# komxun/gym-pybullet-drones-routing

Hardware: AMD Instinct MI355X
Metric: env-steps/sec (drone·dt) at 4096 envs, 1/2/4/8 GPU; state L2 vs PyBullet (higher is better)
Workload: dtype f64; 1 GPU; 4096 HoverAviary envs per GPU (cf2x, Physics.DYN, ActionType.RPM, 240/30 Hz = 8 substeps/step, U[-1,1] actions, SB3 auto-reset); n_envs_per_gpu=4096, global_envs=4096, drones_per_env=1, parallelism=env-sharded x1 (no collective in the step loop)

## Files before the change

### gym_pybullet_drones_routing_amd/csrc/gpd_step_seq.h

```cpp
#pragma once
#include "gpd_step_duo.h"

namespace gpd {


__host__ __device__ inline int seq_rows(int nsub) { return (5 * nsub + 3) | 1; }
__host__ __device__ inline int seq_hand_off_at(int tile_bytes) { return (tile_bytes + 15) & ~15; }
inline size_t seq_lds_bytes(int tile_bytes, int nsub, int tpb, size_t real_bytes) {
  return (size_t)seq_hand_off_at(tile_bytes) + (size_t)2 * 2 * seq_rows(nsub) * tpb * real_bytes;
}

template <typename R, int ACT>
__global__ __launch_bounds__(4 * kWave) void step_seq_kernel(R* __restrict__ state_p, const float* __restrict__ actions_p,
                                                             int2* __restrict__ ctr_p, const Consts<R>* __restrict__ cp,
                                                             long long npad_p, int n_p, int tpb_p, SimView<R> v,
                                                             StepIO<R> io, int n_slots, int slot0, int n_steps,
                                                             int hand_off_at) {
  static_assert(!act_is_pid(ACT), "the fused sequence kernel serves the RPM action types");
  v.state = state_p; v.ctr = ctr_p; v.npad = npad_p; v.N = n_p; v.tpb = tpb_p;
  constexpr int A = act_width(ACT);
  extern __shared__ float4 tile4[];
  float* tilef = reinterpret_cast<float*>(tile4);
  __shared__ unsigned long long sdone[2];
  __shared__ unsigned long long sreset[2];
  __shared__ int shead[kWave];
  const Consts<R>& c = *cp;
  const int tid = threadIdx.x & (kWave - 1);
  const int wave = __builtin_amdgcn_readfirstlane(threadIdx.x) / kWave;
  const long long n0 = (long long)blockIdx.x * v.tpb;
  const long long n = n0 + tid;
  const int nact = (int)((v.N - n0) < v.tpb ? (v.N - n0) : v.tpb);
  const bool active = tid < nact;
  const long long nn = active ? n : n0;
  const long long slot_stride = (long long)v.N * A;
  int slot = slot0;
  auto next_slot = [&]() { slot = slot + 1 == n_slots ? 0 : slot + 1; };
  float nxt[A];
  R* const hbuf = reinterpret_cast<R*>(reinterpret_cast<char*>(tile4) + hand_off_at);
  const int rows = seq_rows(c.nsub);
  const int cstride = v.tpb * rows;
  const int pstride = 2 * cstride;
  const bool own = tid < v.tpb;
  const int lrow = (own ? tid : 0) * rows;

  if (wave == 2) {
    const int L = v.ring_len;
    {
      const float* rb = v.ring + ridx(nn, 0, L, A);
      for (int s = 0; s < L; ++s) {
        const float* src = rb + (long long)s * (64 * A);
        if (A == 4) __builtin_amdgcn_global_load_lds((gbl_void_ptr)src, (lds_void_ptr)(tile4 + s * kPad), 16, 0, 0);
        else __builtin_amdgcn_global_load_lds((gbl_void_ptr)src, (lds_void_ptr)(tilef + s * kPad), 4, 0, 0);
      }
    }
    int hd = v.ctr[nn].y;
    action_load<A>(actions_p + slot * slot_stride, nn, nxt);
    asm volatile("s_waitcnt vmcnt(0)" ::: "memory");
    shead[tid] = hd;
    wave_lds_sync();
    constexpr int U = 4;
    constexpr int EB = A == 4 ? 16 : 4;
    const int total = nact * L;
    const int NC = A == 4 ? 3 + L : v.W;
    const int c0 = A == 4 ? 3 : 12;
    const float rL = 1.0f / (float)L;
    const bool fits = total <= U * kWave;
    const bool wt_rows = (v.wt & 1) != 0;
    const int span = L * kPad;
    float* const dst0 = uniform_ptr(io.obs + n0 * v.W);
    const int nrec = __builtin_amdgcn_readfirstlane(nact * v.W * 4);
    const __amdgpu_buffer_rsrc_t rsrc = __builtin_amdgcn_make_buffer_rsrc(dst0, 0, nrec, 0x00020000);
    int off[U], row[U], idx[U];
#pragma unroll
    for (int u = 0; u < U; ++u) {
      const int g = tid + u * kWave;
      const bool ok = g < total;
      const int gg = ok ? g : total - 1;
      const int i = (int)(((float)gg + 0.5f) * rL), k = gg - i * L;
      int s = shead[i] + 1 + k;
      s -= s >= L ? L : 0;
      s -= s >= L ? L : 0;
      row[u] = i;
      off[u] = ok ? (i * NC + c0 + k) * EB : nrec;
      idx[u] = s * kPad + i;
    }
    int tmod = 0;
    asm volatile("s_barrier" ::: "memory");
    for (int t = 0; t < n_steps; ++t) {
      float a[A];
#pragma unroll
      for (int j = 0; j < A; ++j) a[j] = nxt[j];
      next_slot();
      if (t + 1 < n_steps) action_load<A>(actions_p + slot * slot_stride, nn, nxt);
      if (A == 4) tile4[hd * kPad + tid] = make_float4(a[0], a[1], a[2], a[3]);
      else tilef[hd * kPad + tid] = a[0];
      if (active) ring_append<A>(v.ring, n, hd, L, a);
      wave_lds_sync();
      float4 v4[U];
      float v1[U];
      if (fits) {
#pragma unroll
        for (int u = 0; u < U; ++u) {
          if (A == 4) v4[u] = tile4[idx[u]];
          else v1[u] = tilef[idx[u]];
        }
#pragma unroll
        for (int u = 0; u < U; ++u) {
          if (wt_rows) {
            if (A == 4) store_wt(rsrc, off[u], v4[u]);
            else store_wt(rsrc, off[u], v1[u]);
          } else {
            if (A == 4) __builtin_amdgcn_raw_buffer_store_b128(__builtin_bit_cast(gpd_v4i, v4[u]), rsrc, off[u], 0, 0);
            else __builtin_amdgcn_raw_buffer_store_b32(__builtin_bit_cast(unsigned, v1[u]), rsrc, off[u], 0, 0);
          }
        }
      }
      for (int g = fits ? total : tid; g < total; g += kWave) {
        const int i = (int)(((float)g + 0.5f) * rL), k = g - i * L;
        int s = shead[i] + tmod + 1 + k;
        s -= s >= L ? L : 0;
        s -= s >= L ? L : 0;
        const int o = (i * NC + c0 + k) * EB;
        if (A == 4) {
          const float4 p = tile4[s * kPad + i];
          if (wt_rows) store_wt(rsrc, o, p);
          else __builtin_amdgcn_raw_buffer_store_b128(__builtin_bit_cast(gpd_v4i, p), rsrc, o, 0, 0);
        } else {
          const float p = tilef[s * kPad + i];
          if (wt_rows) store_wt(rsrc, o, p);
          else __builtin_amdgcn_raw_buffer_store_b32(__builtin_bit_cast(unsigned, p), rsrc, o, 0, 0);
        }
      }
      lds_barrier();
      const unsigned long long dr = sdone[t & 1];
      if (dr) {
        float* const tdst = io.terminal_obs + n0 * v.W;
        if (fits) {
#pragma unroll
          for (int u = 0; u < U; ++u) {
            if (tid + u * kWave < total && ((dr >> row[u]) & 1ull)) {
              char* const tp = reinterpret_cast<char*>(tdst) + off[u];
              if (A == 4) *reinterpret_cast<float4*>(tp) = v4[u];
              else *reinterpret_cast<float*>(tp) = v1[u];
            }
          }
        }
        for (int g = fits ? total : tid; g < total; g += kWave) {
          const int i = (int)(((float)g + 0.5f) * rL), k = g - i * L;
          if ((dr >> i) & 1ull) {
            int s = shead[i] + tmod + 1 + k;
            s -= s >= L ? L : 0;
            s -= s >= L ? L : 0;
            const int e = i * NC + c0 + k;
            if (A == 4) reinterpret_cast<float4*>(tdst)[e] = tile4[s * kPad + i];
            else tdst[e] = tilef[s * kPad + i];
          }
        }
      }
      hd = hd + 1 == L ? 0 : hd + 1;
      tmod = tmod + 1 == L ? 0 : tmod + 1;
#pragma unroll
      for (int u = 0; u < U; ++u) {
        idx[u] += kPad;
        idx[u] -= idx[u] >= span ? span : 0;
      }
    }
    return;
  }

  const R* st = v.state + tidx(nn, 0, kStateComps);

  if (wave != 0) {
    const bool from_zero = wave == 3;
    R* const hw = hbuf + (from_zero ? cstride : 0) + lrow;
    if (from_zero) next_slot();
    if (!from_zero || n_steps > 1) action_load<A>(actions_p + slot * slot_stride, nn, nxt);
    R wx = R(0), wy = R(0), wz = R(0);
    if (!from_zero) { wx = st[10 * 64]; wy = st[11 * 64]; wz = st[12 * 64]; }
    DynK<R> dk = dyn_consts(c);
    const int nsub = dk.nsub;
    asm volatile("" : "+v"(wx), "+v"(wy), "+v"(wz));
    auto chain = [&](int u, R* out) {
      float a[A];
#pragma unroll
      for (int j = 0; j < A; ++j) a[j] = nxt[j];
      next_slot();
      if (u + 1 < n_steps) action_load<A>(actions_p + slot * slot_stride, nn, nxt);
      R rpm[4], W[4];
#pragma unroll
      for (int k = 0; k < 4; ++k) rpm[k] = (R)action_to_rpm(dk.hover_f32, a[A == 4 ? k : 0]);
      rpm_wrench<R, 0>(rpm, dk, c, W);
      rate_recur(wx, wy, wz, W, dk);
      for (int k = 0; k < nsub - 1; ++k) {
        R h[5], n2;
        const R cx = wx, cy = wy, cz = wz;
        const bool big = rate_weights(cx, cy, cz, dk, h, n2);
        rate_weights_big(big, n2, dk, h);
        if (own) {
#pragma unroll
          for (int j = 0; j < 5; ++j) out[5 * k + j] = h[j];
        }
        rate_recur(wx, wy, wz, W, dk);
      }
      {
        R h[5], n2;
        const bool big = rate_weights(wx, wy, wz, dk, h, n2);
        rate_weights_big(big, n2, dk, h);
        if (own) {
          R* const o = out + 5 * (nsub - 1);
#pragma unroll
          for (int j = 0; j < 5; ++j) o[j] = h[j];
          o[5] = wx; o[6] = wy; o[7] = wz;
        }
      }
    };
    for (int t = -1; t < n_steps; ++t) {
      if (t + 1 < n_steps && (t >= 0 || !from_zero)) {
        if (from_zero) {
          wx = wy = wz = R(0);
          asm volatile("" : "+v"(wx), "+v"(wy), "+v"(wz));
        } else if (t > 0) {
          if ((sreset[(t - 1) & 1] >> tid) & 1ull) {
            const R* e = hbuf + (t & 1) * pstride + cstride + lrow + 5 * nsub;
            wx = e[0]; wy = e[1]; wz = e[2];
          }
        }
        chain(t + 1, hw + ((t + 1) & 1) * pstride);
      }
      lds_barrier();
    }
    return;
  }

  action_load<A>(actions_p + slot * slot_stride, nn, nxt);
  Drone<R> s;
  R last[4];
  load_drone(v, nn, s, last, false);
  const int2 cv = v.ctr[nn];
  int sc = cv.x;
  int head = cv.y;
  DynK<R> dk = dyn_consts(c, v.task, io.trunc);
  const TailK<R> tk = tail_consts(c, v.bound_xy);
  const int nsub = dk.nsub;
  gpd_global R* st_out = (gpd_global R*)(v.state + tidx(nn, 0, kStateComps));
  int st_off = (int)(tidx(nn, 0, kStateComps) * sizeof(R));
  gpd_global float* rew_out = (gpd_global float*)(io.reward + nn);
  gpd_global uint8_t* term_out = (gpd_global uint8_t*)(io.term + nn);
  gpd_global uint8_t* trunc_out = (gpd_global uint8_t*)(io.trunc + nn);
  gpd_global gpd_v2i* ctr_out = (gpd_global gpd_v2i*)(v.ctr + nn);
  asm volatile("" : "+v"(st_out), "+v"(st_off), "+v"(rew_out), "+v"(term_out), "+v"(trunc_out), "+v"(ctr_out));
  asm volatile("" : "+v"(s.px), "+v"(s.py), "+v"(s.pz), "+v"(s.qx), "+v"(s.qy), "+v"(s.qz), "+v"(s.qw), "+v"(s.vx),
               "+v"(s.vy), "+v"(s.vz), "+v"(sc), "+v"(head));
  const R wnone[3] = {R(0), R(0), R(0)};
  auto hand_off = [&](const R* hp, int k, R h[5]) {
#pragma unroll
    for (int j = 0; j < 5; ++j) h[j] = hp[5 * k + j];
  };
  bool was_reset = false;
  lds_barrier();
  for (int t = 0; t < n_steps; ++t) {
    float a[A];
#pragma unroll
    for (int j = 0; j < A; ++j) a[j] = nxt[j];
    next_slot();
    if (t + 1 < n_steps) action_load<A>(actions_p + slot * slot_stride, nn, nxt);
    R fz;
    {
      R rpm[4], W[4];
#pragma unroll
      for (int k = 0; k < 4; ++k) rpm[k] = (R)action_to_rpm(dk.hover_f32, a[A == 4 ? k : 0]);
      rpm_wrench<R, 0>(rpm, dk, c, W);
      fz = W[0];
#pragma unroll
      for (int k = 0; k < 4; ++k) last[k] = rpm[k];
    }
    const R* const hp = hbuf + (t & 1) * pstride + (was_reset ? cstride : 0) + lrow;
    R h[5];
    hand_off(hp, 0, h);
    if (nsub > 1) {
      R hn[5];
      hand_off(hp, 1, hn);
      pose_half<R, false, true>(s, fz, h, wnone, dk);
      for (int k = 1; k < nsub - 1; ++k) {
#pragma unroll
        for (int j = 0; j < 5; ++j) h[j] = hn[j];
        hand_off(hp, k + 1, hn);
        pose_half<R, false, false>(s, fz, h, wnone, dk);
      }
#pragma unroll
      for (int j = 0; j < 5; ++j) h[j] = hn[j];
    }
    {
      const R* const e = hp + 5 * nsub;
      s.wx = e[0]; s.wy = e[1]; s.wz = e[2];
      const R w[3] = {s.wx, s.wy, s.wz};
      if (nsub > 1) pose_half<R, true, false, true>(s, fz, h, w, dk);
      else pose_half<R, true, true>(s, fz, h, w, dk);
    }
    R qn[4], Rm[9];
    if constexpr (sizeof(R) == 8) readback_fused_rare(s.qx, s.qy, s.qz, s.qw, qn, Rm);
    else readback_fused(s.qx, s.qy, s.qz, s.qw, qn, Rm);
    AttitudeArgs<R> att = attitude_args(qn);
    bool tilted, up_unused;
    attitude_decide<R, true, false>(s.qx, s.qy, s.qz, s.qw, att, tilted, up_unused);
    float roll, pitch, yaw;
    obs_euler_f32(qn, att, roll, pitch, yaw);
    float reward = -1.0f;
    bool term = false, trunc = false;
    if (v.task != TASK_NONE) {
      const R tx = tk.tg[0] - s.px, ty = tk.tg[1] - s.py, tz = tk.tg[2] - s.pz;
      const R d2 = hover_d2(tx, ty, tz);
      R r = R(2) - d2 * d2;
      r = r > R(0) ? r : R(0);
      const bool oob = g_abs(s.px) > tk.bound_xy || g_abs(s.py) > tk.bound_xy || s.pz > R(2) || tilted;
      reward = (float)r;
      term = d2 < R(0.99e-8);
      const bool band = !(d2 < R(0.99e-8)) && !(d2 > R(1.01e-8));
      if (GPD_RARE(__ballot(band) != 0ull)) term = g_sqrt(d2) < R(1e-4);
      trunc = oob || sc >= v.trunc_sc;
    }
    const bool done = term || trunc;
    const bool do_reset = done && v.autoreset;
    float row12[12] = {(float)s.px, (float)s.py, (float)s.pz, roll, pitch, yaw,
                       (float)s.vx, (float)s.vy, (float)s.vz, (float)s.ax, (float)s.ay, (float)s.az};
    if (do_reset) {
      if (active && io.terminal_obs != nullptr) row12_store<A>(io.terminal_obs + n * v.W, row12);
      reset_to_template(tk.ini, s, last, row12);
    }
    const unsigned long long done_rows = __ballot(do_reset && active && io.terminal_obs != nullptr);
    const unsigned long long reset_rows = __ballot(do_reset);
    if (active) {
      if (A == 4) {
        const float4 r0 = make_float4(row12[0], row12[1], row12[2], row12[3]);
        const float4 r1 = make_float4(row12[4], row12[5], row12[6], row12[7]);
        const float4 r2 = make_float4(row12[8], row12[9], row12[10], row12[11]);
        if (v.wt & 1) {
          const __amdgpu_buffer_rsrc_t r =
              __builtin_amdgcn_make_buffer_rsrc(io.obs + n0 * v.W, 0, nact * v.W * 4, 0x00020000);
          const int o = tid * v.W * 4;
          store_wt(r, o, r0); store_wt(r, o + 16, r1); store_wt(r, o + 32, r2);
        } else {
          float4* o4 = reinterpret_cast<float4*>(io.obs + n * v.W);
          o4[0] = r0; o4[1] = r1; o4[2] = r2;
        }
      } else {
        float* orow = io.obs + n * v.W;
#pragma unroll
        for (int k = 0; k < 12; ++k) orow[k] = row12[k];
      }
    }
    if (tid == 0) { sdone[t & 1] = done_rows; sreset[t & 1] = reset_rows; }
    was_reset = do_reset;
    lds_barrier();
    if (active) {
      *rew_out = reward;
      *term_out = (uint8_t)(term ? 1 : 0);
      *trunc_out = (uint8_t)(trunc ? 1 : 0);
    }
    sc = do_reset ? 0 : sc + nsub;
    head = head + 1 == v.ring_len ? 0 : head + 1;
  }
  if (!active) return;
  store_drone_step_at<R, kAuxWt>(v, st_out, st_off, s, last);
  mark_last_in_ring_single(v, n);
  *ctr_out = gpd_v2i{sc, head};
}

}
```

Baseline: 15.01 billion drone*dt/s.

## Offload obs/reward/flag writes to ring wave and reuse precomputed thrust

The pose wave no longer computes Euler angles, builds the observation row, or writes reward/term/trunc. It stages raw state, attitude args and reward in a new double-buffered LDS row buffer, and the ring wave (wave 2) converts and stores them. The thrust fz is now written into the hand-off rows by the rate waves instead of being recomputed from actions in the critical pose wave, and the final rpm is recomputed only once after the loop. This shortens the serial pose-wave chain at the cost of more LDS, another cross-wave dependency and f64-only specialisation.

```diff
diff --git a/gym_pybullet_drones_routing_amd/csrc/gpd_step_seq.h b/gym_pybullet_drones_routing_amd/csrc/gpd_step_seq.h
--- a/gym_pybullet_drones_routing_amd/csrc/gpd_step_seq.h
+++ b/gym_pybullet_drones_routing_amd/csrc/gpd_step_seq.h
@@ -4,10 +4,52 @@
 namespace gpd {
 
 
-__host__ __device__ inline int seq_rows(int nsub) { return (5 * nsub + 3) | 1; }
+__host__ __device__ inline int seq_rows(int nsub) { return (5 * nsub + 4) | 1; }
+constexpr int kSeqRowVals = 18;
 __host__ __device__ inline int seq_hand_off_at(int tile_bytes) { return (tile_bytes + 15) & ~15; }
+__host__ __device__ inline int seq_row_buf_at(int nsub, int tpb) { return 2 * 2 * seq_rows(nsub) * tpb; }
 inline size_t seq_lds_bytes(int tile_bytes, int nsub, int tpb, size_t real_bytes) {
-  return (size_t)seq_hand_off_at(tile_bytes) + (size_t)2 * 2 * seq_rows(nsub) * tpb * real_bytes;
+  return (size_t)seq_hand_off_at(tile_bytes) +
+         ((size_t)seq_row_buf_at(nsub, tpb) + (size_t)2 * kSeqRowVals * tpb) * real_bytes;
+}
+
+__device__ __forceinline__ double seq_rate_n2(double wx, double wy, double wz) {
+#pragma clang fp contract(off)
+  return __builtin_fma(wz, wz, __builtin_fma(wy, wy, wx * wx));
+}
+__device__ __forceinline__ void seq_yaw_args(const double q[4], double& yn, double& yd) {
+#pragma clang fp contract(off)
+  const double x = q[0], y = q[1], z = q[2], w = q[3];
+  yn = 2.0 * __builtin_fma(x, y, w * z);
+  yd = ((w * w + x * x) - y * y) - z * z;
+}
+template <typename R>
+__device__ __forceinline__ bool seq_rate_weights(R wx, R wy, R wz, const DynK<R>& k, R h[5], R& n2) {
+  n2 = seq_rate_n2(wx, wy, wz);
+  const bool rot = n2 > R(1e-16);
+  const R t2 = n2 * k.hdt2;
+  R co, sc;
+  cos_sinc(t2, co, sc);
+  h[0] = co; h[1] = k.hdt * sc;
+  h[2] = rot ? wx : R(0); h[3] = rot ? wy : R(0); h[4] = rot ? wz : R(0);
+  return t2 >= R(0.25);
+}
+
+template <typename R>
+__device__ __forceinline__ void seq_obs_euler_f32(R sarg, R a, R b, R yn, R yd, R x, R y, float& roll, float& pitch,
+                                                  float& yaw) {
+  const bool gimbal = sarg <= R(-0.99999) || sarg >= R(0.99999);
+  const R sa = sarg < R(-1) ? R(-1) : (sarg > R(1) ? R(1) : sarg);
+  pitch = asinf((float)sa);
+  roll = atan2f((float)a, (float)b);
+  yaw = atan2f((float)yn, (float)yd);
+  if (GPD_RARE(__ballot(gimbal) != 0ull)) {
+    if (sarg <= R(-0.99999)) {
+      pitch = -1.57079632679489661923f; roll = 0.0f; yaw = (float)(R(2) * g_atan2(x, -y));
+    } else if (sarg >= R(0.99999)) {
+      pitch = 1.57079632679489661923f; roll = 0.0f; yaw = (float)(R(2) * g_atan2(-x, y));
+    }
+  }
 }
 
 template <typename R, int ACT>
@@ -17,12 +59,15 @@
                                                              StepIO<R> io, int n_slots, int slot0, int n_steps,
                                                              int hand_off_at) {
   static_assert(!act_is_pid(ACT), "the fused sequence kernel serves the RPM action types");
+  static_assert(sizeof(R) == 8, "the fused sequence kernel is built for f64 sims only (gpd.hip, step_seq_fn)");
   v.state = state_p; v.ctr = ctr_p; v.npad = npad_p; v.N = n_p; v.tpb = tpb_p;
   constexpr int A = act_width(ACT);
   extern __shared__ float4 tile4[];
   float* tilef = reinterpret_cast<float*>(tile4);
   __shared__ unsigned long long sdone[2];
   __shared__ unsigned long long sreset[2];
+  __shared__ unsigned long long sterm[2];
+  __shared__ unsigned long long strunc[2];
   __shared__ int shead[kWave];
   const Consts<R>& c = *cp;
   const int tid = threadIdx.x & (kWave - 1);
@@ -42,6 +87,10 @@
   const int pstride = 2 * cstride;
   const bool own = tid < v.tpb;
   const int lrow = (own ? tid : 0) * rows;
+  typedef R R2 __attribute__((ext_vector_type(2)));
+  constexpr int kRowPairs = kSeqRowVals / 2;
+  R2* const rbuf = reinterpret_cast<R2*>(hbuf + seq_row_buf_at(c.nsub, v.tpb)) + (own ? tid : 0) * kRowPairs;
+  const int rpar = v.tpb * kRowPairs;
 
   if (wave == 2) {
     const int L = v.ring_len;
@@ -84,6 +133,8 @@
       off[u] = ok ? (i * NC + c0 + k) * EB : nrec;
       idx[u] = s * kPad + i;
     }
+    float tmpl12[12];
+    row12_from_template(c.init0, tmpl12);
     int tmod = 0;
     asm volatile("s_barrier" ::: "memory");
     for (int t = 0; t < n_steps; ++t) {
@@ -157,6 +208,44 @@
           }
         }
       }
+      {
+        const unsigned long long rs = sreset[t & 1], tm = sterm[t & 1], tr = strunc[t & 1];
+        if (active) {
+          const R2* const rp = rbuf + (t & 1) * rpar;
+          R2 e[kRowPairs];
+#pragma unroll
+          for (int k = 0; k < kRowPairs; ++k) e[k] = rp[k];
+          float roll, pitch, yaw;
+          seq_obs_euler_f32<R>(e[4].y, e[5].x, e[5].y, e[6].x, e[6].y, e[7].x, e[7].y, roll, pitch, yaw);
+          float row12[12] = {(float)e[0].x, (float)e[0].y, (float)e[1].x, roll, pitch, yaw,
+                             (float)e[1].y, (float)e[2].x, (float)e[2].y, (float)e[3].x, (float)e[3].y, (float)e[4].x};
+          const float reward = v.task != TASK_NONE ? (float)e[8].x : -1.0f;
+          if ((rs >> tid) & 1ull) {
+            if ((dr >> tid) & 1ull) row12_store<A>(io.terminal_obs + n * v.W, row12);
+#pragma unroll
+            for (int k = 0; k < 12; ++k) row12[k] = tmpl12[k];
+          }
+          if (A == 4) {
+            const float4 r0 = make_float4(row12[0], row12[1], row12[2], row12[3]);
+            const float4 r1 = make_float4(row12[4], row12[5], row12[6], row12[7]);
+            const float4 r2 = make_float4(row12[8], row12[9], row12[10], row12[11]);
+            if (wt_rows) {
+              const int o = tid * v.W * 4;
+              store_wt(rsrc, o, r0); store_wt(rsrc, o + 16, r1); store_wt(rsrc, o + 32, r2);
+            } else {
+              float4* o4 = reinterpret_cast<float4*>(io.obs + n * v.W);
+              o4[0] = r0; o4[1] = r1; o4[2] = r2;
+            }
+          } else {
+            float* orow = io.obs + n * v.W;
+#pragma unroll
+            for (int k = 0; k < 12; ++k) orow[k] = row12[k];
+          }
+          io.reward[n] = reward;
+          io.term[n] = (uint8_t)((tm >> tid) & 1ull);
+          io.trunc[n] = (uint8_t)((tr >> tid) & 1ull);
+        }
+      }
       hd = hd + 1 == L ? 0 : hd + 1;
       tmod = tmod + 1 == L ? 0 : tmod + 1;
 #pragma unroll
@@ -190,11 +279,12 @@
 #pragma unroll
       for (int k = 0; k < 4; ++k) rpm[k] = (R)action_to_rpm(dk.hover_f32, a[A == 4 ? k : 0]);
       rpm_wrench<R, 0>(rpm, dk, c, W);
+      if (own) out[5 * nsub + 3] = W[0];
       rate_recur(wx, wy, wz, W, dk);
       for (int k = 0; k < nsub - 1; ++k) {
         R h[5], n2;
         const R cx = wx, cy = wy, cz = wz;
-        const bool big = rate_weights(cx, cy, cz, dk, h, n2);
+        const bool big = seq_rate_weights(cx, cy, cz, dk, h, n2);
         rate_weights_big(big, n2, dk, h);
         if (own) {
 #pragma unroll
@@ -204,7 +294,7 @@
       }
       {
         R h[5], n2;
-        const bool big = rate_weights(wx, wy, wz, dk, h, n2);
+        const bool big = seq_rate_weights(wx, wy, wz, dk, h, n2);
         rate_weights_big(big, n2, dk, h);
         if (own) {
           R* const o = out + 5 * (nsub - 1);
@@ -232,7 +322,8 @@
     return;
   }
 
-  action_load<A>(actions_p + slot * slot_stride, nn, nxt);
+  float alast[A];
+  action_load<A>(actions_p + ((slot0 + n_steps - 1) % n_slots) * slot_stride, nn, alast);
   Drone<R> s;
   R last[4];
   load_drone(v, nn, s, last, false);
@@ -244,13 +335,12 @@
   const int nsub = dk.nsub;
   gpd_global R* st_out = (gpd_global R*)(v.state + tidx(nn, 0, kStateComps));
   int st_off = (int)(tidx(nn, 0, kStateComps) * sizeof(R));
-  gpd_global float* rew_out = (gpd_global float*)(io.reward + nn);
-  gpd_global uint8_t* term_out = (gpd_global uint8_t*)(io.term + nn);
-  gpd_global uint8_t* trunc_out = (gpd_global uint8_t*)(io.trunc + nn);
   gpd_global gpd_v2i* ctr_out = (gpd_global gpd_v2i*)(v.ctr + nn);
-  asm volatile("" : "+v"(st_out), "+v"(st_off), "+v"(rew_out), "+v"(term_out), "+v"(trunc_out), "+v"(ctr_out));
+  asm volatile("" : "+v"(st_out), "+v"(st_off), "+v"(ctr_out));
   asm volatile("" : "+v"(s.px), "+v"(s.py), "+v"(s.pz), "+v"(s.qx), "+v"(s.qy), "+v"(s.qz), "+v"(s.qw), "+v"(s.vx),
                "+v"(s.vy), "+v"(s.vz), "+v"(sc), "+v"(head));
+#pragma unroll
+  for (int j = 0; j < A; ++j) asm volatile("" : "+v"(alast[j]));
   const R wnone[3] = {R(0), R(0), R(0)};
   auto hand_off = [&](const R* hp, int k, R h[5]) {
 #pragma unroll
@@ -259,22 +349,8 @@
   bool was_reset = false;
   lds_barrier();
   for (int t = 0; t < n_steps; ++t) {
-    float a[A];
-#pragma unroll
-    for (int j = 0; j < A; ++j) a[j] = nxt[j];
-    next_slot();
-    if (t + 1 < n_steps) action_load<A>(actions_p + slot * slot_stride, nn, nxt);
-    R fz;
-    {
-      R rpm[4], W[4];
-#pragma unroll
-      for (int k = 0; k < 4; ++k) rpm[k] = (R)action_to_rpm(dk.hover_f32, a[A == 4 ? k : 0]);
-      rpm_wrench<R, 0>(rpm, dk, c, W);
-      fz = W[0];
-#pragma unroll
-      for (int k = 0; k < 4; ++k) last[k] = rpm[k];
-    }
     const R* const hp = hbuf + (t & 1) * pstride + (was_reset ? cstride : 0) + lrow;
+    const R fz = hp[5 * nsub + 3];
     R h[5];
     hand_off(hp, 0, h);
     if (nsub > 1) {
@@ -303,9 +379,7 @@
     AttitudeArgs<R> att = attitude_args(qn);
     bool tilted, up_unused;
     attitude_decide<R, true, false>(s.qx, s.qy, s.qz, s.qw, att, tilted, up_unused);
-    float roll, pitch, yaw;
-    obs_euler_f32(qn, att, roll, pitch, yaw);
-    float reward = -1.0f;
+    R rew = R(0);
     bool term = false, trunc = false;
     if (v.task != TASK_NONE) {
       const R tx = tk.tg[0] - s.px, ty = tk.tg[1] - s.py, tz = tk.tg[2] - s.pz;
@@ -313,7 +387,7 @@
       R r = R(2) - d2 * d2;
       r = r > R(0) ? r : R(0);
       const bool oob = g_abs(s.px) > tk.bound_xy || g_abs(s.py) > tk.bound_xy || s.pz > R(2) || tilted;
-      reward = (float)r;
+      rew = r;
       term = d2 < R(0.99e-8);
       const bool band = !(d2 < R(0.99e-8)) && !(d2 > R(1.01e-8));
       if (GPD_RARE(__ballot(band) != 0ull)) term = g_sqrt(d2) < R(1e-4);
@@ -321,46 +395,29 @@
     }
     const bool done = term || trunc;
     const bool do_reset = done && v.autoreset;
-    float row12[12] = {(float)s.px, (float)s.py, (float)s.pz, roll, pitch, yaw,
-                       (float)s.vx, (float)s.vy, (float)s.vz, (float)s.ax, (float)s.ay, (float)s.az};
-    if (do_reset) {
-      if (active && io.terminal_obs != nullptr) row12_store<A>(io.terminal_obs + n * v.W, row12);
-      reset_to_template(tk.ini, s, last, row12);
-    }
+    R yn, yd;
+    seq_yaw_args(qn, yn, yd);
+    if (own) {
+      R2* const rp = rbuf + (t & 1) * rpar;
+      rp[0] = R2{s.px, s.py}; rp[1] = R2{s.pz, s.vx}; rp[2] = R2{s.vy, s.vz};
+      rp[3] = R2{s.ax, s.ay}; rp[4] = R2{s.az, att.sarg}; rp[5] = R2{att.a, att.b};
+      rp[6] = R2{yn, yd};
+      rp[7] = R2{qn[0], qn[1]}; rp[8] = R2{rew, R(0)};
+    }
+    if (do_reset) drone_from_template(tk.ini, s);
     const unsigned long long done_rows = __ballot(do_reset && active && io.terminal_obs != nullptr);
     const unsigned long long reset_rows = __ballot(do_reset);
-    if (active) {
-      if (A == 4) {
-        const float4 r0 = make_float4(row12[0], row12[1], row12[2], row12[3]);
-        const float4 r1 = make_float4(row12[4], row12[5], row12[6], row12[7]);
-        const float4 r2 = make_float4(row12[8], row12[9], row12[10], row12[11]);
-        if (v.wt & 1) {
-          const __amdgpu_buffer_rsrc_t r =
-              __builtin_amdgcn_make_buffer_rsrc(io.obs + n0 * v.W, 0, nact * v.W * 4, 0x00020000);
-          const int o = tid * v.W * 4;
-          store_wt(r, o, r0); store_wt(r, o + 16, r1); store_wt(r, o + 32, r2);
-        } else {
-          float4* o4 = reinterpret_cast<float4*>(io.obs + n * v.W);
-          o4[0] = r0; o4[1] = r1; o4[2] = r2;
-        }
-      } else {
-        float* orow = io.obs + n * v.W;
-#pragma unroll
-        for (int k = 0; k < 12; ++k) orow[k] = row12[k];
-      }
-    }
+    const unsigned long long term_rows = __ballot(term), trunc_rows = __ballot(trunc);
+    if (tid == 0) { sterm[t & 1] = term_rows; strunc[t & 1] = trunc_rows; }
     if (tid == 0) { sdone[t & 1] = done_rows; sreset[t & 1] = reset_rows; }
     was_reset = do_reset;
     lds_barrier();
-    if (active) {
-      *rew_out = reward;
-      *term_out = (uint8_t)(term ? 1 : 0);
-      *trunc_out = (uint8_t)(trunc ? 1 : 0);
-    }
     sc = do_reset ? 0 : sc + nsub;
     head = head + 1 == v.ring_len ? 0 : head + 1;
   }
   if (!active) return;
+#pragma unroll
+  for (int k = 0; k < 4; ++k) last[k] = was_reset ? R(0) : (R)action_to_rpm(dk.hover_f32, alast[A == 4 ? k : 0]);
   store_drone_step_at<R, kAuxWt>(v, st_out, st_off, s, last);
   mark_last_in_ring_single(v, n);
   *ctr_out = gpd_v2i{sc, head};
```

After: 18.10 billion drone*dt/s, median of 6. +20.6%, better.
